# jamesdolezal/biscuit

Measured on AMD Instinct MI355X. Metric: tiles/sec at MC-dropout=30, 299x299x3 (Xception, slide-level pred/sigma reduce), higher is better.
Workload: dtype f16

## Files before the change

### biscuit_amd/csrc/kernels_stream.hip

```cpp
#include "mfma16_common.h"

namespace {
using namespace bqk;

constexpr int STREAM_NW = 12;
constexpr int TAIL_NW = 8;

__device__ __forceinline__ void strip_span(int s, int n, int ns, int& x0, int& nc) {
    const int base = n / ns, rem = n - base * ns;
    x0 = s * base + (s < rem ? s : rem);
    nc = base + (s < rem ? 1 : 0);
}

template <typename T, int NCOL>
struct DwSums {
    f32x2s sa[NCOL], sb[NCOL];
    __device__ __forceinline__ void clear() {
#pragma unroll
        for (int x = 0; x < NCOL; ++x) { sa[x] = (f32x2s){0.f, 0.f}; sb[x] = (f32x2s){0.f, 0.f}; }
    }
    template <bool OUT>
    __device__ __forceinline__ void push(const f32x2s (&tap)[9], const unsigned (&row)[NCOL + 2], unsigned char* a_lane, int ast) {
        f32x2s v[NCOL + 2];
#pragma unroll
        for (int j = 0; j < NCOL + 2; ++j) v[j] = unpack2<T>(row[j]);
#pragma unroll
        for (int x = 0; x < NCOL; ++x) {
            if constexpr (OUT) {
                f32x2s o = sa[x];
#pragma unroll
                for (int dx = 0; dx < 3; ++dx) o = __builtin_elementwise_fma(tap[6 + dx], v[x + dx], o);
                *reinterpret_cast<unsigned*>(a_lane + x * ast) = H16<T>::pack2(o.x, o.y);
            }
            f32x2s a = sb[x];
#pragma unroll
            for (int dx = 0; dx < 3; ++dx) a = __builtin_elementwise_fma(tap[3 + dx], v[x + dx], a);
            sa[x] = a;
            f32x2s b = {0.f, 0.f};
#pragma unroll
            for (int dx = 0; dx < 3; ++dx) b = __builtin_elementwise_fma(tap[dx], v[x + dx], b);
            sb[x] = b;
        }
    }
};

template <typename T, int KS, int NF>
__device__ __forceinline__ void pointwise(const unsigned char* smem_w, const unsigned char* a_read, int lane, f32x4 (&acc)[NF]) {
    constexpr int G = 4, NG = KS * NF / G;
    static_assert(NF % G == 0, "fragments per k-step in groups of four");
#pragma unroll
    for (int f = 0; f < NF; ++f) acc[f] = (f32x4){0.f, 0.f, 0.f, 0.f};
    uint4 b[KS];
#pragma unroll
    for (int ks = 0; ks < KS; ++ks) b[ks] = *reinterpret_cast<const uint4*>(a_read + ks * 64);
    uint4 w[2][G];
    auto fetch = [&](int grp, uint4 (&dst)[G]) {
#pragma unroll
        for (int i = 0; i < G; ++i)
            dst[i] = *reinterpret_cast<const uint4*>(smem_w + ((grp * G + i) * 64 + lane) * 16);
    };
    fetch(0, w[0]);
#pragma unroll
    for (int grp = 0; grp < NG; ++grp) {
        if (grp + 1 < NG) fetch(grp + 1, w[(grp + 1) & 1]);
#pragma unroll
        for (int i = 0; i < G; ++i) {
            const int ks = (grp * G + i) / NF, f = (grp * G + i) % NF;
            acc[f] = mma16<T>(w[grp & 1][i], b[ks], acc[f]);
        }
    }
}

template <typename T>
struct StreamParams {
    const T* in;
    const uint4* wp16;
    const float* dw;
    const float* scale;
    const float* bias;
    T* out;
    int n, H, W;
    int nstrips, nbands;
    int items;
    int relu;
};

template <typename T, int CIN, int COUT, bool RELU_IN, int NW>
__global__ void __launch_bounds__(NW * 64) sepconv_stream_kernel(const StreamParams<T> p) {
    if constexpr (H16<T>::F16) bq_f16_saturate();
    constexpr int NT = NW * 64;
    constexpr int KS = CIN / 32, NF = COUT / 16, NQ = COUT / 32;
    constexpr int HALVES = 128 / CIN;
    constexpr int NCOL = 16 / HALVES;
    constexpr int NWIN = NCOL + 2;
    constexpr int AST = CIN * 2 + 32;
    constexpr int W_BYTES = KS * NF * 1024;
    constexpr int SB_OFF = W_BYTES;
    constexpr int A_OFF = SB_OFF + 2 * COUT * 4;
    constexpr int A_BYTES = 16 * AST;
    static_assert(CIN == 64 || CIN == 128, "lane = channel pair of <= 128 channels");
    extern __shared__ __attribute__((aligned(16))) unsigned char smem[];

    const int tid = threadIdx.x, lane = tid & 63;
    const int wave = __builtin_amdgcn_readfirstlane(tid >> 6);

    for (int i = tid; i < W_BYTES / 16; i += NT) *reinterpret_cast<uint4*>(smem + i * 16) = p.wp16[i];
    for (int i = tid; i < COUT; i += NT) {
        reinterpret_cast<float*>(smem + SB_OFF)[i] = p.scale[i];
        reinterpret_cast<float*>(smem + SB_OFF)[COUT + i] = p.bias[i];
    }
    const int cpair = HALVES == 1 ? lane : (lane & 31);
    const int chalf = HALVES == 1 ? 0 : (lane >> 5);
    f32x2s tap[9];
#pragma unroll
    for (int t = 0; t < 9; ++t) tap[t] = *reinterpret_cast<const f32x2s*>(p.dw + t * CIN + 2 * cpair);
    __syncthreads();

    unsigned char* const At = smem + A_OFF + wave * A_BYTES;
    const int px = lane & 15, g = lane >> 4;
    unsigned char* const a_lane = At + (chalf * NCOL) * AST + cpair * 4;
    const unsigned char* const a_read = At + px * AST + g * 16;
    const float* const sb = reinterpret_cast<const float*>(smem + SB_OFF) + 8 * g;
    const unsigned lo2 = p.relu ? 0u : 0x80008000u;
    const int wgx = xcd_tile(blockIdx.x, gridDim.x);
    const int lane_el = chalf * NCOL * CIN + 2 * cpair;
    const __amdgpu_buffer_rsrc_t orsrc = __builtin_amdgcn_make_buffer_rsrc(
        p.out, 0, (int)((size_t)p.n * p.H * p.W * COUT * sizeof(T)), 0x00020000);

    for (int it = 0;; ++it) {
        const int item = __builtin_amdgcn_readfirstlane((it * (int)gridDim.x + wgx) * NW + wave);
        if (item >= p.items) break;
        const int strip = item % p.nstrips;
        const int t1 = item / p.nstrips;
        const int band = t1 % p.nbands;
        const int img = t1 / p.nbands;
        int x0, nc, y0, nr;
        strip_span(strip, p.W, p.nstrips, x0, nc);
        strip_span(band, p.H, p.nbands, y0, nr);
        const int y1 = y0 + nr;
        const int xl = x0 - 1 + chalf * NCOL;
        unsigned cmask = 0;
#pragma unroll
        for (int j = 0; j < NWIN; ++j) cmask |= ((unsigned)(xl + j) < (unsigned)p.W) ? (1u << j) : 0u;
        const T* const img_in = p.in + ((size_t)img * p.H * p.W + (x0 - 1)) * CIN + lane_el;

        unsigned nx[NWIN], row[NWIN];
        auto load_row = [&](int y) {
            const int yc = y < 0 ? 0 : (y >= p.H ? p.H - 1 : y);
            const T* rp = img_in + (size_t)yc * p.W * CIN;
#pragma unroll
            for (int j = 0; j < NWIN; ++j) nx[j] = *reinterpret_cast<const unsigned*>(rp + j * CIN);
        };
        auto take_row = [&](int y) {
            const unsigned m = (unsigned)y < (unsigned)p.H ? cmask : 0u;
#pragma unroll
            for (int j = 0; j < NWIN; ++j) row[j] = RELU_IN ? relu_pk16(nx[j]) : nx[j];
            if (HALVES == 1 && m == (1u << NWIN) - 1u) return;
            asm volatile("" ::: "memory");
#pragma unroll
            for (int j = 0; j < NWIN; ++j) row[j] = ((m >> j) & 1u) ? row[j] : 0u;
        };
        DwSums<T, NCOL> dws;
        dws.clear();
        load_row(y0 - 1); take_row(y0 - 1);
        load_row(y0);
        dws.template push<false>(tap, row, a_lane, AST);
        take_row(y0);
        load_row(y0 + 1);
        dws.template push<false>(tap, row, a_lane, AST);

        unsigned ooff = px < nc ? (unsigned)(((((size_t)img * p.H + y0) * p.W + x0 + px) * COUT + 8 * g) * sizeof(T)) : 0xfffff000u;
        const unsigned ostep = px < nc ? (unsigned)((size_t)p.W * COUT * sizeof(T)) : 0u;
#pragma unroll
        for (int q = 0; q < NQ; ++q)
            __builtin_amdgcn_raw_buffer_store_b128((u32x4s){0u, 0u, 0u, 0u}, orsrc, (int)(0xfffff000u + 16 * q), 0, 0);
        for (int y = y0; y < y1; ++y, ooff += ostep) {
            take_row(y + 1);
            load_row(y + 2 < y1 ? y + 2 : y1);
            __builtin_amdgcn_sched_barrier(0);
            dws.template push<true>(tap, row, a_lane, AST);
            f32x4 acc[NF];
            pointwise<T, KS, NF>(smem, a_read, lane, acc);
#pragma unroll
            for (int q = 0; q < NQ; ++q) {
                unsigned o[4];
                bn_pair<T>(acc[2 * q], acc[2 * q + 1], sb + 32 * q, COUT, o);
#pragma unroll
                for (int i = 0; i < 4; ++i) asm("v_pk_max_i16 %0, %1, %2" : "=v"(o[i]) : "v"(o[i]), "v"(lo2));
                const u32x4s ov = {o[0], o[1], o[2], o[3]};
                __builtin_amdgcn_raw_buffer_store_b128(ov, orsrc, (int)ooff + 64 * q, 0, 0);
            }
        }
    }
}

template <typename T>
struct TailParams {
    const T* in;
    const uint4* wp16;
    const float* dw;
    const float* scale;
    const float* bias;
    const T* x;
    const uint4* wr16;
    const float* rscale;
    const float* rbias;
    T* out;
    int n, H, W, Ho, Wo;
    int nstrips, nbands, items;
};

__device__ __forceinline__ void band_span(int b, int Ho, int nb, int& p0, int& np) {
    const int base = Ho / nb, rem = Ho - base * nb;
    const int lo = (rem + 1) / 2, hi = rem / 2;
    p0 = b * base + (b < lo ? b : lo) + (b > nb - hi ? b - (nb - hi) : 0);
    np = base + ((b < lo || b >= nb - hi) ? 1 : 0);
}

template <typename T, int CX, int NW>
__global__ void __launch_bounds__(NW * 64) block_tail_stream_kernel(const TailParams<T> p) {
    if constexpr (H16<T>::F16) bq_f16_saturate();
    constexpr int NT = NW * 64;
    constexpr int CIN = 128, COUT = 128, KS = CIN / 32, NF = COUT / 16, NQ = COUT / 32, NCOL = 16, NWIN = NCOL + 2;
    constexpr int KR = CX / 32;
    constexpr int AST = CIN * 2 + 32;
    constexpr int W_BYTES = KS * NF * 1024, WR_BYTES = KR * NF * 1024;
    constexpr int WR_OFF = W_BYTES;
    constexpr int SB_OFF = WR_OFF + WR_BYTES;
    constexpr int A_OFF = SB_OFF + 4 * COUT * 4;
    constexpr int A_BYTES = 16 * AST;
    constexpr unsigned NEG = NegInf<T>::v;
    extern __shared__ __attribute__((aligned(16))) unsigned char smem[];

    const int tid = threadIdx.x, lane = tid & 63;
    const int wave = __builtin_amdgcn_readfirstlane(tid >> 6);
    for (int i = tid; i < W_BYTES / 16; i += NT) *reinterpret_cast<uint4*>(smem + i * 16) = p.wp16[i];
    for (int i = tid; i < WR_BYTES / 16; i += NT) *reinterpret_cast<uint4*>(smem + WR_OFF + i * 16) = p.wr16[i];
    for (int i = tid; i < COUT; i += NT) {
        float* sbw = reinterpret_cast<float*>(smem + SB_OFF);
        sbw[i] = p.scale[i]; sbw[COUT + i] = p.bias[i]; sbw[2 * COUT + i] = p.rscale[i]; sbw[3 * COUT + i] = p.rbias[i];
    }
    f32x2s tap[9];
#pragma unroll
    for (int t = 0; t < 9; ++t) tap[t] = *reinterpret_cast<const f32x2s*>(p.dw + t * CIN + 2 * lane);
    __syncthreads();

    unsigned char* const At = smem + A_OFF + wave * A_BYTES;
    const int px = lane & 15, g = lane >> 4;
    unsigned char* const a_lane = At + lane * 4;
    const unsigned char* const a_read = At + px * AST + g * 16;
    const float* const sb = reinterpret_cast<const float*>(smem + SB_OFF) + 8 * g;
    const int wgx = xcd_tile(blockIdx.x, gridDim.x);
    const int pt = p.H & 1, pl = p.W & 1;
    const __amdgpu_buffer_rsrc_t orsrc = __builtin_amdgcn_make_buffer_rsrc(
        p.out, 0, (int)((size_t)p.n * p.Ho * p.Wo * COUT * sizeof(T)), 0x00020000);

    for (int it = 0;; ++it) {
        const int item = __builtin_amdgcn_readfirstlane((it * (int)gridDim.x + wgx) * NW + wave);
        if (item >= p.items) break;
        const int strip = item % p.nstrips;
        const int t1 = item / p.nstrips;
        const int band = t1 % p.nbands;
        const int img = t1 / p.nbands;
        int xo_a, npx, p0, npb;
        strip_span(strip, p.Wo, p.nstrips, xo_a, npx);
        band_span(band, p.Ho, p.nbands, p0, npb);
        const int x0 = 2 * xo_a - pl;
        int ys = 2 * p0 - pt;
        int ye = 2 * (p0 + npb - 1) - pt + 2;
        ys = ys < 0 ? 0 : ys;
        ye = ye > p.H - 1 ? p.H - 1 : ye;
        const int xl = x0 - 1;
        unsigned cmask = 0;
#pragma unroll
        for (int j = 0; j < NWIN; ++j) cmask |= ((unsigned)(xl + j) < (unsigned)p.W) ? (1u << j) : 0u;
        const T* const img_in = p.in + ((size_t)img * p.H * p.W + (x0 - 1)) * CIN + 2 * lane;
        const bool col_out = (unsigned)(x0 + px) >= (unsigned)p.W;
        const bool any_col_out = x0 < 0 || x0 + 15 >= p.W;
        int xs = x0 + (px | 1) - (1 - pl);
        xs = xs < 0 ? 0 : (xs > p.W - 1 ? p.W - 1 : xs);
        const T* const xcol = p.x + ((size_t)img * p.H * p.W + xs) * CX + 8 * g;
        const bool lane_out = (px & 1) && (px >> 1) < npx;
        const unsigned obase = (unsigned)((((size_t)img * p.Ho * p.Wo + xo_a + (px >> 1)) * COUT + 8 * g) * sizeof(T));

        unsigned nx[NWIN], row[NWIN];
        auto load_row = [&](int y) {
            const int yc = y < 0 ? 0 : (y >= p.H ? p.H - 1 : y);
            const T* rp = img_in + (size_t)yc * p.W * CIN;
#pragma unroll
            for (int j = 0; j < NWIN; ++j) nx[j] = *reinterpret_cast<const unsigned*>(rp + j * CIN);
        };
        auto take_row = [&](int y) {
            const unsigned m = (unsigned)y < (unsigned)p.H ? cmask : 0u;
#pragma unroll
            for (int j = 0; j < NWIN; ++j) row[j] = nx[j];
            if (m == (1u << NWIN) - 1u) return;
            asm volatile("" ::: "memory");
#pragma unroll
            for (int j = 0; j < NWIN; ++j) row[j] = ((m >> j) & 1u) ? row[j] : 0u;
        };
        DwSums<T, NCOL> dws;
        dws.clear();
        load_row(ys - 1); take_row(ys - 1);
        load_row(ys);
        dws.template push<false>(tap, row, a_lane, AST);
        take_row(ys);
        load_row(ys + 1);
        dws.template push<false>(tap, row, a_lane, AST);

        unsigned VM[4 * NQ];
#pragma unroll
        for (int i = 0; i < 4 * NQ; ++i) VM[i] = NEG;
#pragma unroll
        for (int q = 0; q < NQ; ++q)
            __builtin_amdgcn_raw_buffer_store_b128((u32x4s){0u, 0u, 0u, 0u}, orsrc, (int)(0xfffff000u + 16 * q), 0, 0);

        for (int y = ys; y <= ye; ++y) {
            const int t = y + pt;
            const bool t_even = (t & 1) == 0;
            int yo = (t - 1) >> 1;
            yo = yo < 0 ? 0 : (yo > p.Ho - 1 ? p.Ho - 1 : yo);
            const bool do_emit = (t_even ? t >= 2 : y == p.H - 1) && yo >= p0 && y <= ye;
            take_row(y + 1);
            uint4 xb[KR];
            {
                const T* xr = xcol + (size_t)(2 * yo) * p.W * CX;
#pragma unroll
                for (int ks = 0; ks < KR; ++ks) xb[ks] = *reinterpret_cast<const uint4*>(xr + 32 * ks);
            }
            load_row(y + 2 <= ye + 1 ? y + 2 : ye + 1);
            __builtin_amdgcn_sched_barrier(0);
            dws.template push<true>(tap, row, a_lane, AST);
            f32x4 acc[NF];
            pointwise<T, KS, NF>(smem, a_read, lane, acc);
            unsigned cur[4 * NQ];
#pragma unroll
            for (int q = 0; q < NQ; ++q) {
                unsigned o[4];
                bn_pair<T>(acc[2 * q], acc[2 * q + 1], sb + 32 * q, COUT, o);
#pragma unroll
                for (int i = 0; i < 4; ++i) cur[4 * q + i] = o[i];
            }
            if (any_col_out) {
                asm volatile("" ::: "memory");
#pragma unroll
                for (int i = 0; i < 4 * NQ; ++i) cur[i] = col_out ? NEG : cur[i];
            }
#pragma unroll
            for (int i = 0; i < 4 * NQ; ++i) VM[i] = pmax2<T>(VM[i], cur[i]);
            u32x4s po[NQ];
#pragma unroll
            for (int q = 0; q < NQ; ++q) po[q] = (u32x4s){0u, 0u, 0u, 0u};
            if (do_emit) {
                asm volatile("" ::: "memory");
                f32x4 ar[NF];
#pragma unroll
                for (int f = 0; f < NF; ++f) ar[f] = (f32x4){0.f, 0.f, 0.f, 0.f};
#pragma unroll
                for (int ks = 0; ks < KR; ++ks)
#pragma unroll
                    for (int f = 0; f < NF; ++f) {
                        const uint4 wf = *reinterpret_cast<const uint4*>(smem + WR_OFF + ((ks * NF + f) * 64 + lane) * 16);
                        ar[f] = mma16<T>(wf, xb[ks], ar[f]);
                    }
#pragma unroll
                for (int q = 0; q < NQ; ++q) {
                    unsigned res[4], o[4];
                    bn_pair<T>(ar[2 * q], ar[2 * q + 1], sb + 2 * COUT + 32 * q, COUT, res);
#pragma unroll
                    for (int i = 0; i < 4; ++i) {
                        const unsigned c = VM[4 * q + i];
                        const unsigned lft = (unsigned)__builtin_amdgcn_mov_dpp((int)c, 0x111, 0xf, 0xf, true);
                        const unsigned rgt = (unsigned)__builtin_amdgcn_mov_dpp((int)c, 0x101, 0xf, 0xf, true);
                        o[i] = padd2<T>(pmax2<T>(pmax2<T>(lft, c), rgt), res[i]);
                    }
                    po[q] = (u32x4s){o[0], o[1], o[2], o[3]};
                }
            }
            {
                const unsigned off = (do_emit && lane_out) ? obase + (unsigned)yo * (unsigned)(p.Wo * COUT * sizeof(T)) : 0xfffff000u;
#pragma unroll
                for (int q = 0; q < NQ; ++q)
                    __builtin_amdgcn_raw_buffer_store_b128(po[q], orsrc, (int)off + 64 * q, 0, 0);
            }
            if (t_even) {
#pragma unroll
                for (int i = 0; i < 4 * NQ; ++i) VM[i] = cur[i];
            }
        }
    }
}

inline int pick_bands(long long base_items, int rows, int rows_per_band, int min_rows, int waves);

template <typename T>
struct CoopParams {
    const T* in;
    const uint4* wp16;
    const float* dw;
    const float* scale;
    const float* bias;
    const T* x;
    const uint4* wr16;
    const float* rscale;
    const float* rbias;
    T* out;
    int n, H, W, Ho, Wo;
    int nstrips, nbands, items;
};

template <typename T, int C, int WGS>
__global__ void __launch_bounds__(C * 2, WGS) block_tail_coop_kernel(const CoopParams<T> p) {
    if constexpr (H16<T>::F16) bq_f16_saturate();
    constexpr int CIN = C, COUT = C, CX = C / 2, KS = CIN / 32, KR = CX / 32, NCOL = 4, NWIN = NCOL + 2;
    constexpr int NT = C * 2, NFR = COUT / 16;
    constexpr int AST = CIN * 2 + 32;
    constexpr int A_BYTES = 16 * AST;
    constexpr int SB_OFF = 2 * A_BYTES;
    constexpr unsigned NEG = NegInf<T>::v;
    extern __shared__ __attribute__((aligned(16))) unsigned char smem[];

    const int tid = threadIdx.x, lane = tid & 63;
    const int wave = __builtin_amdgcn_readfirstlane(tid >> 6);
    for (int i = tid; i < COUT; i += NT) {
        float* sbw = reinterpret_cast<float*>(smem + SB_OFF);
        sbw[i] = p.scale[i]; sbw[COUT + i] = p.bias[i]; sbw[2 * COUT + i] = p.rscale[i]; sbw[3 * COUT + i] = p.rbias[i];
    }
    uint4 wq[KS][2], wrq[KR][2];
#pragma unroll
    for (int ks = 0; ks < KS; ++ks)
#pragma unroll
        for (int i = 0; i < 2; ++i) wq[ks][i] = p.wp16[((size_t)ks * NFR + 2 * wave + i) * 64 + lane];
#pragma unroll
    for (int ks = 0; ks < KR; ++ks)
#pragma unroll
        for (int i = 0; i < 2; ++i) wrq[ks][i] = p.wr16[((size_t)ks * NFR + 2 * wave + i) * 64 + lane];
    const int pair = lane & 15, cg = lane >> 4;
    f32x2s tap[9];
#pragma unroll
    for (int t = 0; t < 9; ++t) tap[t] = *reinterpret_cast<const f32x2s*>(p.dw + t * CIN + 32 * wave + 2 * pair);
    __syncthreads();

    const int px = lane & 15, g = lane >> 4;
    const float* const sb = reinterpret_cast<const float*>(smem + SB_OFF) + 32 * wave + 8 * g;
    const int wgx = xcd_tile(blockIdx.x, gridDim.x);
    const int pt = p.H & 1, pl = p.W & 1;
    const __amdgpu_buffer_rsrc_t orsrc = __builtin_amdgcn_make_buffer_rsrc(
        p.out, 0, (int)((size_t)p.n * p.Ho * p.Wo * COUT * sizeof(T)), 0x00020000);

    for (int item = wgx; item < p.items; item += (int)gridDim.x) {
        const int strip = item % p.nstrips;
        const int t1 = item / p.nstrips;
        const int band = t1 % p.nbands;
        const int img = t1 / p.nbands;
        int xo_a, npx, p0, npb;
        strip_span(strip, p.Wo, p.nstrips, xo_a, npx);
        band_span(band, p.Ho, p.nbands, p0, npb);
        const int x0 = 2 * xo_a - pl;
        int ys = 2 * p0 - pt;
        int ye = 2 * (p0 + npb - 1) - pt + 2;
        ye = ye > p.H - 1 ? p.H - 1 : ye;
        const int xl = x0 - 1 + NCOL * cg;
        unsigned cmask = 0;
#pragma unroll
        for (int j = 0; j < NWIN; ++j) cmask |= ((unsigned)(xl + j) < (unsigned)p.W) ? (1u << j) : 0u;
        const bool inner = x0 >= 1 && x0 + 16 < p.W;
        const T* const img_in = p.in + ((size_t)img * p.H * p.W + xl) * CIN + 32 * wave + 2 * pair;
        const bool col_out = (unsigned)(x0 + px) >= (unsigned)p.W;
        const bool any_col_out = x0 < 0 || x0 + 15 >= p.W;
        int xs = x0 + (px | 1) - (1 - pl);
        xs = xs < 0 ? 0 : (xs > p.W - 1 ? p.W - 1 : xs);
        const T* const xcol = p.x + ((size_t)img * p.H * p.W + xs) * CX + 8 * g;
        const bool lane_out = (px & 1) && (px >> 1) < npx;
        const unsigned obase = (unsigned)((((size_t)img * p.Ho * p.Wo + xo_a + (px >> 1)) * COUT + 32 * wave + 8 * g) * sizeof(T));

        unsigned nxA[NWIN], nxB[NWIN], row[NWIN];
        auto load_row = [&](int y, unsigned (&nx)[NWIN]) {
            const int yc = y < 0 ? 0 : (y >= p.H ? p.H - 1 : y);
            const T* rp = img_in + (size_t)yc * p.W * CIN;
#pragma unroll
            for (int j = 0; j < NWIN; ++j) nx[j] = *reinterpret_cast<const unsigned*>(rp + j * CIN);
        };
        auto take_row = [&](int y, const unsigned (&nx)[NWIN]) {
            const unsigned m = (unsigned)y < (unsigned)p.H ? cmask : 0u;
#pragma unroll
            for (int j = 0; j < NWIN; ++j) row[j] = nx[j];
            if (inner && (unsigned)y < (unsigned)p.H) return;
            asm volatile("" ::: "memory");
#pragma unroll
            for (int j = 0; j < NWIN; ++j) row[j] = ((m >> j) & 1u) ? row[j] : 0u;
        };
        DwSums<T, NCOL> dws;
        dws.clear();
        unsigned char* a_lane0 = smem + (NCOL * cg) * AST + (32 * wave + 2 * pair) * 2;
        uint4 xb[KR];
        auto load_x = [&](int yo) {
            const T* xr = xcol + (size_t)(2 * yo) * p.W * CX;
#pragma unroll
            for (int ks = 0; ks < KR; ++ks) xb[ks] = *reinterpret_cast<const uint4*>(xr + 32 * ks);
        };
        load_x(p0);
        load_row(ys - 1, nxA); load_row(ys, nxB);
        take_row(ys - 1, nxA); load_row(ys + 1, nxA);
        dws.template push<false>(tap, row, a_lane0, AST);
        take_row(ys, nxB); load_row(ys + 2, nxB);
        dws.template push<false>(tap, row, a_lane0, AST);
        take_row(ys + 1, nxA); load_row(ys + 3, nxA);
        dws.template push<true>(tap, row, a_lane0, AST);
        asm volatile("s_waitcnt lgkmcnt(0)\n\ts_barrier" ::: "memory");

        unsigned VM[4];
#pragma unroll
        for (int i = 0; i < 4; ++i) VM[i] = NEG;
#pragma unroll
        for (int i = 0; i < 6; ++i)
            __builtin_amdgcn_raw_buffer_store_b128((u32x4s){0u, 0u, 0u, 0u}, orsrc, (int)(0xfffff000u + 16u * i), 0, 0);
        auto step = [&](int y, int buf, unsigned (&nx)[NWIN], auto parity) {
            const int t = y + pt;
            constexpr bool t_even = decltype(parity)::value;
            int yo = (t - 1) >> 1;
            yo = yo < 0 ? 0 : (yo > p.Ho - 1 ? p.Ho - 1 : yo);
            const bool do_emit = (t_even ? t >= 2 : y == p.H - 1) && yo >= p0 && y <= ye;
            take_row(y + 2, nx);
            load_row(y + 4 <= ye + 2 ? y + 4 : ye + 2, nx);
            __builtin_amdgcn_sched_barrier(0);
            f32x4 acc[2] = {{0.f, 0.f, 0.f, 0.f}, {0.f, 0.f, 0.f, 0.f}};
            {
                const unsigned char* ar = smem + buf * A_BYTES + px * AST + g * 16;
                uint4 b[KS];
#pragma unroll
                for (int ks = 0; ks < KS; ++ks) b[ks] = *reinterpret_cast<const uint4*>(ar + ks * 64);
#pragma unroll
                for (int ks = 0; ks < KS; ++ks)
#pragma unroll
                    for (int i = 0; i < 2; ++i) acc[i] = mma16<T>(wq[ks][i], b[ks], acc[i]);
            }
            dws.template push<true>(tap, row, a_lane0 + (buf ^ 1) * A_BYTES, AST);
            unsigned cur[4];
            bn_pair<T>(acc[0], acc[1], sb, COUT, cur);
            if (any_col_out || y < 0) {
                asm volatile("" ::: "memory");
#pragma unroll
                for (int i = 0; i < 4; ++i) cur[i] = (col_out || y < 0) ? NEG : cur[i];
            }
#pragma unroll
            for (int i = 0; i < 4; ++i) VM[i] = pmax2<T>(VM[i], cur[i]);
            u32x4s po = {0u, 0u, 0u, 0u};
            if (do_emit) {
                asm volatile("" ::: "memory");
                f32x4 ar[2] = {{0.f, 0.f, 0.f, 0.f}, {0.f, 0.f, 0.f, 0.f}};
#pragma unroll
                for (int ks = 0; ks < KR; ++ks)
#pragma unroll
                    for (int i = 0; i < 2; ++i) ar[i] = mma16<T>(wrq[ks][i], xb[ks], ar[i]);
                unsigned res[4];
                bn_pair<T>(ar[0], ar[1], sb + 2 * COUT, COUT, res);
#pragma unroll
                for (int i = 0; i < 4; ++i) {
                    const unsigned c = VM[i];
                    const unsigned lft = (unsigned)__builtin_amdgcn_mov_dpp((int)c, 0x111, 0xf, 0xf, true);
                    const unsigned rgt = (unsigned)__builtin_amdgcn_mov_dpp((int)c, 0x101, 0xf, 0xf, true);
                    po[i] = padd2<T>(pmax2<T>(pmax2<T>(lft, c), rgt), res[i]);
                }
            }
            {
                const unsigned off = (do_emit && lane_out) ? obase + (unsigned)yo * (unsigned)(p.Wo * COUT * sizeof(T)) : 0xfffff000u;
                __builtin_amdgcn_raw_buffer_store_b128(po, orsrc, (int)off, 0, 0);
            }
            if constexpr (t_even) {
                load_x((t >> 1) > p.Ho - 1 ? p.Ho - 1 : (t >> 1));
#pragma unroll
                for (int i = 0; i < 4; ++i) VM[i] = cur[i];
            }
            asm volatile("s_waitcnt lgkmcnt(0)\n\ts_barrier" ::: "memory");
        };
        for (int y = ys; y <= ye; y += 2) {
            step(y, 0, nxB, std::true_type{});
            step(y + 1, 1, nxA, std::false_type{});
        }
    }
}

template <typename T, int C, int WGS>
int launch_coop(CoopParams<T> p, int num_cus, hipStream_t s) {
    constexpr size_t lds = 2 * 16 * (C * 2 + 32) + 4 * C * 4;
    auto kern = block_tail_coop_kernel<T, C, WGS>;
    static BqLdsAttr attr;
    if (const int e = attr.ensure(reinterpret_cast<const void*>(kern), lds)) return e;
    p.Ho = (p.H + 1) / 2; p.Wo = (p.W + 1) / 2;
    p.nstrips = (p.Wo + 6) / 7;
    const long long base_items = (long long)p.n * p.nstrips;
    p.nbands = pick_bands(base_items, p.Ho, p.Ho, 2, num_cus * WGS);
    p.items = (int)(base_items * p.nbands);
    int grid = p.items < num_cus * WGS ? p.items : num_cus * WGS;
    hipLaunchKernelGGL(kern, dim3(grid), dim3(C * 2), lds, s, p);
    return (int)hipGetLastError();
}

inline int pick_bands(long long base_items, int rows, int rows_per_band, int min_rows, int waves) {
    int nb = (rows + rows_per_band - 1) / rows_per_band;
    if (base_items * nb < waves) {
        nb = (int)((waves + base_items - 1) / base_items);
        if (nb > rows / min_rows) nb = rows / min_rows;
        if (nb < 1) nb = 1;
    }
    return nb;
}

template <typename T, int CIN, int COUT, bool RELU_IN>
int launch_stream(StreamParams<T> p, int num_cus, hipStream_t s) {
    constexpr int NW = COUT > 128 ? 8 : STREAM_NW;
    constexpr size_t lds = (size_t)(CIN / 32) * (COUT / 16) * 1024 + 2 * COUT * 4 + (size_t)NW * 16 * (CIN * 2 + 32);
    static_assert(lds <= 160 * 1024, "stream kernel LDS budget");
    auto kern = sepconv_stream_kernel<T, CIN, COUT, RELU_IN, NW>;
    static BqLdsAttr attr;
    if (const int e = attr.ensure(reinterpret_cast<const void*>(kern), lds)) return e;
    p.nstrips = (p.W + 15) / 16;
    const long long base_items = (long long)p.n * p.nstrips;
    p.nbands = p.H <= 80 ? pick_bands(base_items, p.H, 10, 4, num_cus * NW) : pick_bands(base_items, p.H, 25, 4, num_cus * NW);
    p.items = (int)(base_items * p.nbands);
    int grid = (p.items + NW - 1) / NW;
    if (grid > num_cus) grid = num_cus;
    hipLaunchKernelGGL(kern, dim3(grid), dim3(NW * 64), lds, s, p);
    return (int)hipGetLastError();
}

template <typename T, int CX>
int launch_tail(TailParams<T> p, int num_cus, hipStream_t s) {
    constexpr int NW = TAIL_NW;
    constexpr size_t lds = (size_t)4 * 8 * 1024 + (size_t)(CX / 32) * 8 * 1024 + 4 * 128 * 4 + (size_t)NW * 16 * (128 * 2 + 32);
    static_assert(lds <= 160 * 1024, "tail kernel LDS budget");
    auto kern = block_tail_stream_kernel<T, CX, NW>;
    static BqLdsAttr attr;
    if (const int e = attr.ensure(reinterpret_cast<const void*>(kern), lds)) return e;
    p.Ho = (p.H + 1) / 2; p.Wo = (p.W + 1) / 2;
    p.nstrips = (p.Wo + 6) / 7;
    const long long base_items = (long long)p.n * p.nstrips;
    p.nbands = pick_bands(base_items, p.Ho, 18, 2, num_cus * NW);
    p.items = (int)(base_items * p.nbands);
    int grid = (p.items + NW - 1) / NW;
    if (grid > num_cus) grid = num_cus;
    hipLaunchKernelGGL(kern, dim3(grid), dim3(NW * 64), lds, s, p);
    return (int)hipGetLastError();
}

template <typename T>
int launch_stream_t(int cin, int cout, bool relu_in, const void* in, const void* wp16, const float* dw, const float* scale,
                    const float* bias, void* out, int n, int H, int W, int relu, int num_cus, hipStream_t s) {
    StreamParams<T> p;
    p.in = reinterpret_cast<const T*>(in);
    p.wp16 = reinterpret_cast<const uint4*>(wp16);
    p.dw = dw; p.scale = scale; p.bias = bias;
    p.out = reinterpret_cast<T*>(out);
    p.n = n; p.H = H; p.W = W; p.relu = relu;
    p.nstrips = p.nbands = p.items = 0;
    if (cin == 64 && cout == 128 && !relu_in) return launch_stream<T, 64, 128, false>(p, num_cus, s);
    if (cin == 128 && cout == 128 && !relu_in) return launch_stream<T, 128, 128, false>(p, num_cus, s);
    if (cin == 128 && cout == 256 && relu_in) return launch_stream<T, 128, 256, true>(p, num_cus, s);
    return (int)hipErrorInvalidValue;
}

}

bool stream_supported(int dtype, int cin, int cout, bool relu_in, long long n, int H, int W) {
    const bool b2 = !relu_in && cout == 128 && (cin == 64 || cin == 128);
    const bool b3 = relu_in && cout == 256 && cin == 128;
    return dtype != 0 && (b2 || b3) && H >= 4 && W >= 1 &&
           n * H * W * (long long)cout * 2 <= 0xfffff000ll;
}

bool tail_supported(int dtype, int cin, int cout, int cx, long long n, int H, int W) {
    const bool b2 = cin == 128 && cout == 128 && cx == 64;
    const bool b3 = cin == 256 && cout == 256 && cx == 128;
    return dtype != 0 && (b2 || b3) && H >= 8 && W >= 8 &&
           n * H * W * (long long)cin * 2 <= 0xfffff000ll;
}

int launch_block_tail(int dtype, int cin, int cout, int cx, const void* y1, const void* wp16, const float* dw,
                      const float* scale, const float* bias, const void* x, const void* wr16, const float* rscale,
                      const float* rbias, void* out, int n, int H, int W, int num_cus, hipStream_t s) {
    if (!tail_supported(dtype, cin, cout, cx, n, H, W)) return (int)hipErrorInvalidValue;
    if (cin == 256) {
        auto go3 = [&](auto tag) {
            typedef decltype(tag) T;
            CoopParams<T> p;
            p.in = reinterpret_cast<const T*>(y1); p.wp16 = reinterpret_cast<const uint4*>(wp16); p.dw = dw;
            p.scale = scale; p.bias = bias;
            p.x = reinterpret_cast<const T*>(x); p.wr16 = reinterpret_cast<const uint4*>(wr16); p.rscale = rscale; p.rbias = rbias;
            p.out = reinterpret_cast<T*>(out);
            p.n = n; p.H = H; p.W = W; p.Ho = p.Wo = p.nstrips = p.nbands = p.items = 0;
            return launch_coop<T, 256, 1>(p, num_cus, s);
        };
        return dtype == 2 ? go3(f16_t{}) : go3(bf16_t{});
    }
    auto go = [&](auto tag) {
        typedef decltype(tag) T;
        TailParams<T> p;
        p.in = reinterpret_cast<const T*>(y1); p.wp16 = reinterpret_cast<const uint4*>(wp16); p.dw = dw;
        p.scale = scale; p.bias = bias;
        p.x = reinterpret_cast<const T*>(x); p.wr16 = reinterpret_cast<const uint4*>(wr16); p.rscale = rscale; p.rbias = rbias;
        p.out = reinterpret_cast<T*>(out);
        p.n = n; p.H = H; p.W = W; p.Ho = p.Wo = p.nstrips = p.nbands = p.items = 0;
        return launch_tail<T, 64>(p, num_cus, s);
    };
    return dtype == 2 ? go(f16_t{}) : go(bf16_t{});
}

int launch_sepconv_stream(int dtype, int cin, int cout, bool relu_in, const void* in, const void* wp16, const float* dw,
                          const float* scale, const float* bias, void* out, int n, int H, int W, int relu, int num_cus,
                          hipStream_t s) {
    return dtype == 2 ? launch_stream_t<f16_t>(cin, cout, relu_in, in, wp16, dw, scale, bias, out, n, H, W, relu, num_cus, s)
                      : launch_stream_t<bf16_t>(cin, cout, relu_in, in, wp16, dw, scale, bias, out, n, H, W, relu, num_cus, s);
}
```

Baseline: 33820.

## Use buffer loads, inline-asm pool/max, and hoisted unpack in stream kernels

```diff
diff --git a/biscuit_amd/csrc/kernels_stream.hip b/biscuit_amd/csrc/kernels_stream.hip
--- a/biscuit_amd/csrc/kernels_stream.hip
+++ b/biscuit_amd/csrc/kernels_stream.hip
@@ -24,6 +24,10 @@
         f32x2s v[NCOL + 2];
 #pragma unroll
         for (int j = 0; j < NCOL + 2; ++j) v[j] = unpack2<T>(row[j]);
+        push_f32<OUT>(tap, v, a_lane, ast);
+    }
+    template <bool OUT>
+    __device__ __forceinline__ void push_f32(const f32x2s (&tap)[9], const f32x2s (&v)[NCOL + 2], unsigned char* a_lane, int ast) {
 #pragma unroll
         for (int x = 0; x < NCOL; ++x) {
             if constexpr (OUT) {
@@ -43,6 +47,36 @@
         }
     }
 };
+
+template <typename T>
+__device__ __forceinline__ unsigned pool_add(unsigned l, unsigned c, unsigned r, unsigned res) {
+    return padd2<T>(pmax2<T>(pmax2<T>(l, c), r), res);
+}
+template <>
+__device__ __forceinline__ unsigned pool_add<f16_t>(unsigned l, unsigned c, unsigned r, unsigned res) {
+    unsigned d, m;
+    float lo, hi;
+    asm("v_pk_max_f16 %1, %4, %5\n\t"
+        "v_pk_max_f16 %1, %1, %6\n\t"
+        "v_fma_mix_f32 %2, %1, 1.0, %7 op_sel_hi:[1,0,1]\n\t"
+        "v_fma_mix_f32 %3, %1, 1.0, %7 op_sel:[1,0,1] op_sel_hi:[1,0,1]\n\t"
+        "v_cvt_pk_f16_f32 %0, %2, %3"
+        : "=v"(d), "=&v"(m), "=&v"(lo), "=&v"(hi) : "v"(l), "v"(c), "v"(r), "v"(res));
+    return d;
+}
+template <typename T>
+__device__ __forceinline__ void pmax2x4(unsigned* a, const unsigned* b) {
+#pragma unroll
+    for (int i = 0; i < 4; ++i) a[i] = pmax2<T>(a[i], b[i]);
+}
+template <>
+__device__ __forceinline__ void pmax2x4<f16_t>(unsigned* a, const unsigned* b) {
+    asm("v_pk_max_f16 %0, %0, %4\n\t"
+        "v_pk_max_f16 %1, %1, %5\n\t"
+        "v_pk_max_f16 %2, %2, %6\n\t"
+        "v_pk_max_f16 %3, %3, %7"
+        : "+v"(a[0]), "+v"(a[1]), "+v"(a[2]), "+v"(a[3]) : "v"(b[0]), "v"(b[1]), "v"(b[2]), "v"(b[3]));
+}
 
 template <typename T, int KS, int NF>
 __device__ __forceinline__ void pointwise(const unsigned char* smem_w, const unsigned char* a_read, int lane, f32x4 (&acc)[NF]) {
@@ -254,6 +288,11 @@
     const int pt = p.H & 1, pl = p.W & 1;
     const __amdgpu_buffer_rsrc_t orsrc = __builtin_amdgcn_make_buffer_rsrc(
         p.out, 0, (int)((size_t)p.n * p.Ho * p.Wo * COUT * sizeof(T)), 0x00020000);
+    const __amdgpu_buffer_rsrc_t irsrc = __builtin_amdgcn_make_buffer_rsrc(
+        const_cast<T*>(p.in), 0, (int)((size_t)p.n * p.H * p.W * CIN * sizeof(T)), 0x00020000);
+    const __amdgpu_buffer_rsrc_t xrsrc = __builtin_amdgcn_make_buffer_rsrc(
+        const_cast<T*>(p.x), 0, (int)((size_t)p.n * p.H * p.W * CX * sizeof(T)), 0x00020000);
+    const unsigned row_bytes = (unsigned)(p.W * CIN * sizeof(T)), xrow_bytes = (unsigned)(2 * p.W * CX * sizeof(T));
 
     for (int it = 0;; ++it) {
         const int item = __builtin_amdgcn_readfirstlane((it * (int)gridDim.x + wgx) * NW + wave);
@@ -274,39 +313,45 @@
         unsigned cmask = 0;
 #pragma unroll
         for (int j = 0; j < NWIN; ++j) cmask |= ((unsigned)(xl + j) < (unsigned)p.W) ? (1u << j) : 0u;
-        const T* const img_in = p.in + ((size_t)img * p.H * p.W + (x0 - 1)) * CIN + 2 * lane;
+        const unsigned ib0 = (unsigned)((((size_t)img * p.H * p.W + (x0 - 1)) * CIN + 2 * lane) * sizeof(T));
+        const unsigned ib2 = ib0 + 2u * CIN * sizeof(T);
         const bool col_out = (unsigned)(x0 + px) >= (unsigned)p.W;
         const bool any_col_out = x0 < 0 || x0 + 15 >= p.W;
         int xs = x0 + (px | 1) - (1 - pl);
         xs = xs < 0 ? 0 : (xs > p.W - 1 ? p.W - 1 : xs);
-        const T* const xcol = p.x + ((size_t)img * p.H * p.W + xs) * CX + 8 * g;
+        const unsigned xcol = (unsigned)((((size_t)img * p.H * p.W + xs) * CX + 8 * g) * sizeof(T));
         const bool lane_out = (px & 1) && (px >> 1) < npx;
         const unsigned obase = (unsigned)((((size_t)img * p.Ho * p.Wo + xo_a + (px >> 1)) * COUT + 8 * g) * sizeof(T));
 
-        unsigned nx[NWIN], row[NWIN];
+        unsigned nx[NWIN];
+        f32x2s v[NWIN];
         auto load_row = [&](int y) {
             const int yc = y < 0 ? 0 : (y >= p.H ? p.H - 1 : y);
-            const T* rp = img_in + (size_t)yc * p.W * CIN;
-#pragma unroll
-            for (int j = 0; j < NWIN; ++j) nx[j] = *reinterpret_cast<const unsigned*>(rp + j * CIN);
+            const unsigned ro = (unsigned)yc * row_bytes;
+#pragma unroll
+            for (int j = 0; j < 2; ++j) nx[j] = __builtin_amdgcn_raw_buffer_load_b32(irsrc, (int)(ib0 + ro), j * CIN * (int)sizeof(T), 0);
+#pragma unroll
+            for (int j = 2; j < NWIN; ++j)
+                nx[j] = __builtin_amdgcn_raw_buffer_load_b32(irsrc, (int)(ib2 + ro), (j - 2) * CIN * (int)sizeof(T), 0);
         };
         auto take_row = [&](int y) {
             const unsigned m = (unsigned)y < (unsigned)p.H ? cmask : 0u;
-#pragma unroll
-            for (int j = 0; j < NWIN; ++j) row[j] = nx[j];
-            if (m == (1u << NWIN) - 1u) return;
-            asm volatile("" ::: "memory");
-#pragma unroll
-            for (int j = 0; j < NWIN; ++j) row[j] = ((m >> j) & 1u) ? row[j] : 0u;
+            if (m != (1u << NWIN) - 1u) {
+                asm volatile("" ::: "memory");
+#pragma unroll
+                for (int j = 0; j < NWIN; ++j) nx[j] = ((m >> j) & 1u) ? nx[j] : 0u;
+            }
+#pragma unroll
+            for (int j = 0; j < NWIN; ++j) v[j] = unpack2<T>(nx[j]);
         };
         DwSums<T, NCOL> dws;
         dws.clear();
         load_row(ys - 1); take_row(ys - 1);
         load_row(ys);
-        dws.template push<false>(tap, row, a_lane, AST);
+        dws.template push_f32<false>(tap, v, a_lane, AST);
         take_row(ys);
         load_row(ys + 1);
-        dws.template push<false>(tap, row, a_lane, AST);
+        dws.template push_f32<false>(tap, v, a_lane, AST);
 
         unsigned VM[4 * NQ];
 #pragma unroll
@@ -324,13 +369,14 @@
             take_row(y + 1);
             uint4 xb[KR];
             {
-                const T* xr = xcol + (size_t)(2 * yo) * p.W * CX;
-#pragma unroll
-                for (int ks = 0; ks < KR; ++ks) xb[ks] = *reinterpret_cast<const uint4*>(xr + 32 * ks);
+                const unsigned xo = xcol + (unsigned)yo * xrow_bytes;
+#pragma unroll
+                for (int ks = 0; ks < KR; ++ks)
+                    xb[ks] = __builtin_bit_cast(uint4, __builtin_amdgcn_raw_buffer_load_b128(xrsrc, (int)xo, 64 * ks, 0));
             }
             load_row(y + 2 <= ye + 1 ? y + 2 : ye + 1);
             __builtin_amdgcn_sched_barrier(0);
-            dws.template push<true>(tap, row, a_lane, AST);
+            dws.template push_f32<true>(tap, v, a_lane, AST);
             f32x4 acc[NF];
             pointwise<T, KS, NF>(smem, a_read, lane, acc);
             unsigned cur[4 * NQ];
@@ -347,10 +393,10 @@
                 for (int i = 0; i < 4 * NQ; ++i) cur[i] = col_out ? NEG : cur[i];
             }
 #pragma unroll
-            for (int i = 0; i < 4 * NQ; ++i) VM[i] = pmax2<T>(VM[i], cur[i]);
+            for (int q = 0; q < NQ; ++q) pmax2x4<T>(VM + 4 * q, cur + 4 * q);
             u32x4s po[NQ];
 #pragma unroll
-            for (int q = 0; q < NQ; ++q) po[q] = (u32x4s){0u, 0u, 0u, 0u};
+            for (int q = 0; q < NQ; ++q) po[q] = __builtin_nondeterministic_value(po[q]);
             if (do_emit) {
                 asm volatile("" ::: "memory");
                 f32x4 ar[NF];
@@ -372,7 +418,7 @@
                         const unsigned c = VM[4 * q + i];
                         const unsigned lft = (unsigned)__builtin_amdgcn_mov_dpp((int)c, 0x111, 0xf, 0xf, true);
                         const unsigned rgt = (unsigned)__builtin_amdgcn_mov_dpp((int)c, 0x101, 0xf, 0xf, true);
-                        o[i] = padd2<T>(pmax2<T>(pmax2<T>(lft, c), rgt), res[i]);
+                        o[i] = pool_add<T>(lft, c, rgt, res[i]);
                     }
                     po[q] = (u32x4s){o[0], o[1], o[2], o[3]};
                 }
@@ -543,9 +589,9 @@
 #pragma unroll
                 for (int i = 0; i < 4; ++i) cur[i] = (col_out || y < 0) ? NEG : cur[i];
             }
-#pragma unroll
-            for (int i = 0; i < 4; ++i) VM[i] = pmax2<T>(VM[i], cur[i]);
-            u32x4s po = {0u, 0u, 0u, 0u};
+            pmax2x4<T>(VM, cur);
+            u32x4s po;
+            po = __builtin_nondeterministic_value(po);
             if (do_emit) {
                 asm volatile("" ::: "memory");
                 f32x4 ar[2] = {{0.f, 0.f, 0.f, 0.f}, {0.f, 0.f, 0.f, 0.f}};
@@ -560,7 +606,7 @@
                     const unsigned c = VM[i];
                     const unsigned lft = (unsigned)__builtin_amdgcn_mov_dpp((int)c, 0x111, 0xf, 0xf, true);
                     const unsigned rgt = (unsigned)__builtin_amdgcn_mov_dpp((int)c, 0x101, 0xf, 0xf, true);
-                    po[i] = padd2<T>(pmax2<T>(pmax2<T>(lft, c), rgt), res[i]);
+                    po[i] = pool_add<T>(lft, c, rgt, res[i]);
                 }
             }
             {
```

Measured after the change: 33930 (median of 6 runs). About the same (+0.3%).
